# 0xC0000054/pdn-jpegxl

Hardware: AMD Instinct MI355X
Metric: megapixels/sec decode (4K lossy VarDCT) (higher is better)
Workload: dtype f32

## Files before the change

### pdn_jpegxl_amd/csrc/decoder.cc

```cpp
#include <hip/hip_runtime.h>
#include <algorithm>
#include <atomic>
#include <cmath>
#include <cstdarg>
#include <cstdio>
#include <cstdlib>
#include <cstring>
#include <memory>
#include <mutex>
#include <string>
#include <thread>
#include <vector>
#include "../../include/jxlfiletypeio.h"
#include "batch_layout.h"
#include "entropy_plan.h"
#include "host_parse.h"
#include "icc.h"
#include "kernels.h"

namespace jxlhip {

struct HipError : std::runtime_error {
  explicit HipError(const std::string& m) : std::runtime_error(m) {}
};
// ... 65 lines not shown
    std::vector<int> parse_status;
    std::vector<std::string> parse_msg;
    std::vector<size_t> status_off;
    DevImage* d_imgs = nullptr;
    bool pending = false;
    hipEvent_t lf_done = nullptr, hf_done = nullptr, done = nullptr, uploaded = nullptr;
    std::vector<Tap> taps;
    std::vector<std::string> stage_names;
    std::vector<int> stage_chain;
    std::vector<hipEvent_t> events;
    std::vector<float> stage_ms;
  };
  static constexpr int kSlots = 3;
  static constexpr int kPixelChunk = 32;
  Slot slots[kSlots];
  int cur = 0, last = 0;
  Slot* active = &slots[0];
  hipStream_t stream_lf = nullptr;
  hipStream_t stream_hf = nullptr;
  hipStream_t last_stream = nullptr;
  std::vector<std::string> total_names;
  std::vector<double> total_ms;
  int total_batches = 0;
  std::string sticky_error;
  int sticky_status = 0;
  uint8_t* li_dev = nullptr; uint8_t* li_host = nullptr; size_t li_cap = 0;
  void EnsureLoadImageBuffers(size_t bytes);
  int lane_stride_override = 0;
  int hf_stride_override = 0;
  bool debug_taps = false;
  int band_first_row = 0, band_rows = 0;
  bool no_stream_pairs = false;
  bool no_lf_pipeline = false;
  int alpha_narrow_limit = 32767;
  bool no_direct = false, mod_lanes64 = false;
  bool overlap = true;
  int downscale = 1;

  explicit JxlHipDecoder(int dev);
  ~JxlHipDecoder();
  void EnsureWs(size_t bytes);
  void EnsureBlob(size_t bytes);
  void Mark(const char* name, hipStream_t s, int chain);
  void WaitSlot(Slot& S);
  Slot& Last() { return slots[last]; }
  void Decode(int32_t n_, const uint8_t* const* host_data, const size_t* sizes, const uint8_t* const* dev_data,
              uint8_t* const* dev_out, hipStream_t stream, bool sync, DecoderStatus* statuses, ErrorInfo* err);
  DecoderStatus Finish(DecoderStatus* statuses, ErrorInfo* err);
  void CopyPlaneTap(int stage);
  void PrepassSingle(ParsedFrame& f, const uint8_t* dev_file);
  EntropyPlanOptions PlanOptions() const;
};

JxlHipDecoder::JxlHipDecoder(int dev) {
  if (dev < 0) HIP_OK(hipGetDevice(&dev));
  device = dev;
  HIP_OK(hipSetDevice(device));
  int entropy_cus = 0, pixel_cus = 0;
  if (const char* e = Knob("JXLHIP_ENTROPY_CUS")) entropy_cus = std::min(256, std::max(0, atoi(e)));
  if (const char* e = Knob("JXLHIP_PIXEL_CUS")) pixel_cus = std::min(256, std::max(0, atoi(e)));
  auto masked_stream = [](hipStream_t* s, int first, int count) {
    uint32_t mask[8] = {0, 0, 0, 0, 0, 0, 0, 0};
    for (int i = first; i < first + count; i++) mask[i >> 5] |= 1u << (i & 31);
    HIP_OK(hipExtStreamCreateWithCUMask(s, 8, mask));
  };
  if (pixel_cus) masked_stream(&own_stream, 256 - pixel_cus, pixel_cus);
// ... 398 lines not shown
  if (any_alpha && !(skip_stages & 4))
    LaunchAlphaAns(d_imgs, B.alpha_tasks, nalpha_t, plan.alpha_stride, plan.alpha.Bytes(), plan.direct_alpha, plan.lean_mod,
                   alpha_narrow, s_hf);
  if (!ds || any_alpha) Mark("alpha_ans", s_hf, 1);
  if (debug_taps && !ds) {
    taps.assign(n, Tap());
    LaunchExpandCoefficients(d_imgs, n, true, B.max_tiles, stream);
    HIP_OK(hipStreamSynchronize(stream));
    CopyPlaneTap(0);
  }
  const bool finish_on_hf = s_hf == stream || debug_taps || !Knob("JXLHIP_ALPHA_FINISH_ON_PIX");
  if (finish_on_hf) {
    if (any_alpha && !(skip_stages & 4)) LaunchAlphaFinish(d_imgs, n, max_groups, alpha_narrow > 0, s_hf);
    if (!ds || any_alpha) Mark("alpha_finish", s_hf, 1);
  }
  if (s_hf != stream) {
    HIP_OK(hipEventRecord(S.hf_done, s_hf));
    HIP_OK(hipStreamWaitEvent(stream, S.hf_done, 0));
  }
  Mark("main_start", stream, 2);
  if (!finish_on_hf) {
    if (any_alpha && !(skip_stages & 4)) LaunchAlphaFinish(d_imgs, n, max_groups, alpha_narrow > 0, stream);
    Mark("alpha_finish", stream, 2);
  }
  hipStream_t s_pix = pix_on_hf ? s_hf : stream;
  if (ds && B.any_vardct) {
    if (any_alpha) LaunchAlphaReduce(d_imgs, n, B.max_ds_cells, s_pix);
    LaunchLfOutput(d_imgs, n, B.max_ds_cells, s_pix);
    Mark("lf_output", s_pix, 2);
  }
  for (int c0 = 0; c0 < (ds ? 0 : n); c0 += pixel_chunk) {
    const int cnt = std::min(pixel_chunk, n - c0);
    if (!(skip_stages & 8))
    LaunchReconTiles(d_imgs + c0, cnt, B.max_tiles, d_basis_all, d_basis_small, d_llf_scale, d_basis_mfma, s_pix);
    Mark("reconstruct", s_pix, 2);
    LaunchExpandCoefficients(d_imgs + c0, cnt, false, B.max_tiles, s_pix);
    LaunchGenericReconstruct(d_imgs + c0, cnt, d_basis_all, d_basis_small, d_llf_scale, s_pix);
    Mark("reconstruct_generic", s_pix, 2);
    if (debug_taps) { HIP_OK(hipStreamSynchronize(s_pix)); CopyPlaneTap(1); }
    if (any_noise && !(early_noise && c0 == 0)) { LaunchNoise(d_imgs + c0, cnt, max_groups, B.max_w, B.max_h, s_pix); Mark("noise", s_pix, 2); }
    if (!(skip_stages & 16))
    LaunchFilterTiles(d_imgs + c0, cnt, B.max_w, B.max_h, B.stage_mask, B.any_unfiltered, B.any_fused, B.any_fused2, s_pix);
    Mark("filters+output", s_pix, 2);
  }
  if (s_pix != stream) {
    HIP_OK(hipEventRecord(S.hf_done, s_pix));
    HIP_OK(hipStreamWaitEvent(stream, S.hf_done, 0));
  }
  if (nmod_t) {
    if (s_lf != stream) { HIP_OK(hipEventRecord(S.lf_done, s_lf)); HIP_OK(hipStreamWaitEvent(stream, S.lf_done, 0)); }
    LaunchModularAns(d_imgs, n, B.mod_tasks, nmod_t, plan.mod.Bytes(), plan.max_mod_groups,
                     plan.max_mod_coded, plan.mod_lanes, plan.mod_rb, plan.mod_wp_lds, plan.direct_mod, stream);
    for (auto& op : B.mod_ops) {
      if (op.kind == 3) LaunchModularPalette(op.a, op.b, op.out, op.nout, op.type, op.rw, op.rh, op.status, stream);
      else LaunchModularOp(op.kind, op.a, op.b, op.c, op.aw, op.ah, op.rw, op.rh, op.type, stream);
    }
    LaunchModularOut(d_imgs, n, B.max_mod_pixels, stream);
    if (ds) LaunchBoxReduce(d_imgs, n, B.max_ds_cells, stream);
    Mark("modular", stream, 2);
  }
  if (!patches.tiles.empty()) {
    LaunchPatches(B.patch_frames, B.patch_tiles, (int)patches.tiles.size(), B.patch_list, B.patch_pos, B.patch_refs, stream);
    Mark("patches", stream, 2);
  }
  if (!comps.empty()) {
    LaunchCompose(B.comp_imgs, B.comp_frames, (int)comps.size(), B.max_segments, stream);
    Mark("compose", stream, 2);
// ... 203 lines not shown
    return DecoderStatus_DecodeError;
  }
}

DecoderStatus jxlhip_finish(JxlHipDecoder* dec, DecoderStatus* statuses, ErrorInfo* err) {
  if (!dec) return DecoderStatus_NullParameter;
  try {
    return dec->Finish(statuses, err);
  } catch (const std::exception& e) {
    SetErr(err, "%s", e.what());
    return DecoderStatus_DecodeError;
  }
}

int32_t jxlhip_set_option(JxlHipDecoder* dec, const char* name, int32_t value) {
  if (!dec || !name) return 0;
  if (!strcmp(name, "debug_taps")) { dec->debug_taps = value != 0; return 1; }
  if (!strcmp(name, "query_pixel_chunk")) return JxlHipDecoder::kPixelChunk;
  if (!strcmp(name, "lane_stride")) { if (value != 0 && !PowerOfTwoUpTo64(value)) return 0; dec->lane_stride_override = value; return 1; }
  if (!strcmp(name, "band_first_row")) { if (value < 0) return 0; dec->band_first_row = value; return 1; }
  if (!strcmp(name, "band_rows")) { if (value < 0) return 0; dec->band_rows = value; return 1; }
  if (!strcmp(name, "no_direct")) { dec->no_direct = value != 0; return 1; }
  if (!strcmp(name, "alpha_narrow_limit")) { if (value < 0 || value > 32767) return 0; dec->alpha_narrow_limit = value; return 1; }
  if (!strcmp(name, "query_alpha_narrow_groups") || !strcmp(name, "query_alpha_redo_groups")) {
    JxlHipDecoder::Slot& S = dec->Last();
    if (S.pending || !S.h_status) return -1;
    const int word = name[12] == 'n' ? kStatusAlphaNarrow : kStatusAlphaRedo;
    int64_t sum = 0;
    for (int i = 0; i < S.n; i++) sum += S.h_status[(size_t)i * 16 + word];
    return (int32_t)std::min<int64_t>(sum, INT32_MAX);
  }
  if (!strcmp(name, "no_stream_pairs")) { dec->no_stream_pairs = value != 0; return 1; }
  if (!strcmp(name, "no_lf_pipeline")) { dec->no_lf_pipeline = value != 0; return 1; }
  if (!strcmp(name, "mod_lanes64")) { dec->mod_lanes64 = value != 0; return 1; }
  if (!strcmp(name, "overlap")) { dec->overlap = value != 0; return 1; }
  if (!strcmp(name, "downscale")) { if (value != 1 && value != 8) return 0; dec->downscale = value; return 1; }
  return 0;
}

size_t jxlhip_read_plane(JxlHipDecoder* dec, int32_t index, const char* name, int32_t channel, void* dst, size_t capacity) {
  if (!dec || !name) return 0;
  JxlHipDecoder::Slot& S = dec->Last();
  if (index < 0 || index >= S.n || S.pending) return 0;
  if (S.parse_status[index] != DecoderStatus_Ok) return 0;
  const DevImage& d = S.imgs[index];
  std::string nm(name);
  const size_t cells = (size_t)d.w8 * d.h8, pix = (size_t)d.wp * d.hp;
  const void* src = nullptr;
  size_t bytes = 0;
  bool host = false;
  const int c = std::min(2, std::max(0, channel));
  if (nm == "lf") { src = d.lf_final[c]; bytes = cells * 4; }
  else if (nm == "lf_quant") { src = d.lfq[c]; bytes = cells * 4; }
  else if (nm == "cellinfo") { src = d.cellinfo; bytes = cells * 4; }
  else if (nm == "raw_quant") { src = d.rawq; bytes = cells * 2; }
  else if (nm == "sharpness") { src = d.sharp; bytes = cells; }
  else if (nm == "ytox") { src = d.ytox; bytes = (size_t)d.wt * d.ht; }
  else if (nm == "ytob") { src = d.ytob; bytes = (size_t)d.wt * d.ht; }
  else if (nm == "alpha") { src = d.alpha; bytes = (size_t)d.w * d.h; }
  else if (nm == "inv_sigma") { src = d.inv_sigma; bytes = cells * 4; }
  else if (dec->debug_taps && (size_t)index < S.taps.size()) {
    host = true;
    if (nm == "qcoef") { src = S.taps[index].qcoef[c].data(); bytes = S.taps[index].qcoef[c].size(); }
    else if (nm == "xyb_idct") { src = S.taps[index].xyb_idct[c].data(); bytes = S.taps[index].xyb_idct[c].size(); }
    else if (nm == "xyb_filtered") { src = S.taps[index].xyb_filtered[c].data(); bytes = S.taps[index].xyb_filtered[c].size(); }
    else if (nm == "noise_rnd") { src = S.taps[index].noise_rnd[c].data(); bytes = S.taps[index].noise_rnd[c].size(); }
// ... 230 lines not shown
```

### pdn_jpegxl_amd/csrc/kernels.h

```cpp
#pragma once
#include <hip/hip_runtime.h>
#include "dev_types.h"

namespace jxlhip {

void LaunchLfAns(const DevImage* imgs, const SectionTask* tasks, int ntasks, int slots, size_t lds_bytes, int scalar_rows, bool lean, hipStream_t s);
void LaunchLfFinish(const DevImage* imgs, const SectionTask* tasks, int ntasks, bool pipeline, hipStream_t s);
void LaunchHfBlockList(const DevImage* imgs, int nimg, int max_groups, hipStream_t s);
void LaunchHfDecode(const DevImage* imgs, const SectionTask* tasks, int nwg, int threads, int lane_stride, size_t lds_bytes, size_t lane_bytes,
                    hipStream_t s);
void LaunchAlphaAns(const DevImage* imgs, const SectionTask* tasks, int nwg, int lane_stride, size_t lds_bytes, int scalar_rows, bool lean, int narrow_limit,
                    hipStream_t s);
void LaunchAlphaFinish(const DevImage* imgs, int nimg, int max_groups, bool narrow, hipStream_t s);
void LaunchModularAns(const DevImage* imgs, int nimg, const SectionTask* tasks, int ntasks, size_t lds_bytes, int max_sections, int max_coded,
                      int lanes, int rb_width, int wp_lds, int scalar_rows, hipStream_t s);
void LaunchModularOp(int kind, int32_t* a, int32_t* b, int32_t* c, int aw, int ah, int rw, int rh, int type, hipStream_t s);
void LaunchModularPalette(const int32_t* palette, const int32_t* index, int32_t* const* out, int nout, int nb_colors, int w, int h, uint32_t* status,
                          hipStream_t s);
void LaunchModularOut(const DevImage* imgs, int nimg, size_t max_pixels, hipStream_t s);
void LaunchOrient(const uint8_t* src, uint8_t* dst, int w, int h, int px_bytes, int orientation, hipStream_t s);
void LaunchLfPixelStages(const DevImage* imgs, int nimg, size_t max_cells, hipStream_t s);
void LaunchExpandCoefficients(const DevImage* imgs, int nimg, bool all_tiles, int max_tiles, hipStream_t s);
void LaunchGenericReconstruct(const DevImage* imgs, int nimg, const float* basis_all, const float* basis_small,
                              const float* llf_scale, hipStream_t s);
void LaunchReconTiles(const DevImage* imgs, int nimg, int max_tiles, const float* basis_all, const float* basis_small,
                      const float* llf_scale, const float* basis_mfma, hipStream_t s);
void LaunchFilterTiles(const DevImage* imgs, int nimg, int max_w, int max_h, int stage_mask, bool any_unfiltered,
                       int any_fused, int any_fused2, hipStream_t s);

void LaunchLfOutput(const DevImage* imgs, int nimg, size_t max_cells, hipStream_t s);
void LaunchAlphaReduce(const DevImage* imgs, int nimg, size_t max_cells, hipStream_t s);
void LaunchBoxReduce(const DevImage* imgs, int nimg, size_t max_cells, hipStream_t s);

void LaunchNoise(const DevImage* imgs, int nimg, int max_groups, int max_w, int max_h, hipStream_t s);

void LaunchCompose(const ComposeImage* imgs, const ComposeFrame* frames, int nimg, int max_segments, hipStream_t s);
void LaunchPatches(const PatchFrame* frames, const PatchTile* tiles, int ntiles, const int32_t* list, const PatchPos* pos, const PatchRef* refs,
                   hipStream_t s);

void LaunchStatusToHost(const uint32_t* src, uint32_t* dst_pinned, int nwords, hipStream_t s);
#ifdef JXLHIP_EXPERIMENTS
void LaunchInterference(int kind, int wg_per_cu, int lds_kb, float ms, float* scratch, size_t scratch_bytes, hipStream_t s);
#endif

}
```

### pdn_jpegxl_amd/csrc/tile_kernels.hip

```cpp
#include <hip/hip_runtime.h>
#include <cstdlib>
#include "dev_types.h"
#include "dev_util.h"
#include "kernels.h"

namespace jxlhip {

#ifndef JXLHIP_PRIO_PIXEL
#define JXLHIP_PRIO_PIXEL 0
#endif
#if JXLHIP_PRIO_PIXEL
#define JXL_PIXEL_PRIO() __builtin_amdgcn_s_setprio(JXLHIP_PRIO_PIXEL)
#else
#define JXL_PIXEL_PRIO() ((void)0)
#endif

namespace {

constexpr int kTS = 64;
constexpr int kLP = 65;

__device__ const uint8_t t_quant_table[kNumStrategies] = {0, 1, 2, 3, 4, 5, 6, 6, 7, 7, 8, 8, 9, 9, 10, 10, 10, 10, 11, 12, 12, 13, 14, 14, 15, 16, 16};

__device__ __forceinline__ bool Special(uint32_t s) { return (s >= 1 && s <= 3) || (s >= 12 && s <= 17); }
typedef float __attribute__((ext_vector_type(4))) F4;
template <int N>
__device__ __forceinline__ F4 MfmaChain(const float* pa, int sa, const float* pb, int sb) {
  float a[N / 4], b[N / 4];
#pragma unroll
  for (int k = 0; k < N / 4; k++) { a[k] = pa[k * sa]; b[k] = pb[k * sb]; }
  F4 acc = {0.f, 0.f, 0.f, 0.f};
#pragma unroll
  for (int k = 0; k < N / 4; k++) acc = __builtin_amdgcn_mfma_f32_16x16x4f32(a[k], b[k], acc, 0, 0, 0);
  return acc;
}
template <bool kTableIsA>
__device__ __forceinline__ F4 MfmaChain32L(const float4* t_lo, const float4* t_hi, int pair, const float* po, int so) {
  const float4 v0 = t_lo[pair], v1 = t_hi[pair];
  const float t[8] = {v0.x, v0.y, v0.z, v0.w, v1.x, v1.y, v1.z, v1.w};
  float o[8];
#pragma unroll
  for (int k = 0; k < 8; k++) o[k] = po[k * so];
  F4 acc = {0.f, 0.f, 0.f, 0.f};
#pragma unroll
  for (int k = 0; k < 8; k++)
    acc = kTableIsA ? __builtin_amdgcn_mfma_f32_16x16x4f32(t[k], o[k], acc, 0, 0, 0) : __builtin_amdgcn_mfma_f32_16x16x4f32(o[k], t[k], acc, 0, 0, 0);
  return acc;
}
template <bool kTableIsA>
__device__ __forceinline__ F4 MfmaChain64L(const float4* t64, int pair, const float* po, int so) {
  float t[16], o[16];
#pragma unroll
  for (int j = 0; j < 4; j++) {
    const float4 v = t64[j * 256 + pair];
    t[4 * j] = v.x; t[4 * j + 1] = v.y; t[4 * j + 2] = v.z; t[4 * j + 3] = v.w;
  }
#pragma unroll
  for (int k = 0; k < 16; k++) o[k] = po[k * so];
  F4 acc = {0.f, 0.f, 0.f, 0.f};
#pragma unroll
  for (int k = 0; k < 16; k++)
    acc = kTableIsA ? __builtin_amdgcn_mfma_f32_16x16x4f32(t[k], o[k], acc, 0, 0, 0) : __builtin_amdgcn_mfma_f32_16x16x4f32(o[k], t[k], acc, 0, 0, 0);
  return acc;
}
__device__ __forceinline__ bool MfmaRows(uint32_t tl, uint32_t tr) {
  return (tl >> 31) && (tr >> 31) && ((tl >> 21) & 7) >= 1 && ((tl >> 21) & 7) == ((tr >> 21) & 7) && ((tl >> 13) & 31) == ((tr >> 13) & 31);
}
__device__ __forceinline__ bool MfmaCols(uint32_t tl, uint32_t bl) {
  return (tl >> 31) && (bl >> 31) && ((tl >> 18) & 7) >= 1 && ((tl >> 18) & 7) == ((bl >> 18) & 7) && ((tl >> 8) & 31) == ((bl >> 8) & 31);
}

__device__ __forceinline__ float SrgbOetfT(float v) {
  const float lin = 12.92f * v;
  const float cur = 1.055f * __builtin_amdgcn_exp2f(__builtin_amdgcn_logf(v) * (1.0f / 2.4f)) - 0.055f;
  return v <= 0.0031308f ? lin : cur;
}
__device__ __forceinline__ float SrgbOetf255T(float v) {
  const float lin = (12.92f * 255.0f) * v;
  const float cur = (1.055f * 255.0f) * __builtin_amdgcn_exp2f(__builtin_amdgcn_logf(v) * (1.0f / 2.4f)) - (0.055f * 255.0f);
  return v <= 0.0031308f ? lin : cur;
}
__device__ __forceinline__ float PowT(float a, float e) { return __builtin_amdgcn_exp2f(__builtin_amdgcn_logf(a) * e); }
__device__ __forceinline__ float EncodeTransferT(int kind, float v, float pq_scale, const float* lut = nullptr) {
  if (kind == 0) return v;
  if (kind == 5) {
    const float t = __builtin_sqrtf(fminf(fmaxf(v, 0.f), 1.f)) * 4095.0f;
    const int i = min((int)t, 4094);
    return lut[i] + (lut[i + 1] - lut[i]) * (t - (float)i);
  }
  const float a = fabsf(v);
  float r;
  if (kind == 1) r = a <= 0.0031308f ? 12.92f * a : 1.055f * PowT(a, 1.0f / 2.4f) - 0.055f;
  else if (kind == 2) r = a < 0.018f ? 4.5f * a : 1.099f * PowT(a, 0.45f) - 0.099f;
  else {
    const float xp = a > 0.f ? PowT(a * pq_scale, 0.1593017578125f) : 0.f;
// ... 104 lines not shown
    }
  }
  WritePixelA(im, x, y, X, Y, B, a);
}
__device__ __forceinline__ void WritePixel(const DevImage& im, int x, int y, float X, float Y, float B) {
  const uint32_t a = im.has_alpha ? LoadAlpha(im, (size_t)y * im.w + x) : 0u;
  if (im.has_noise) { WritePixelGeneral(im, x, y, X, Y, B, a); return; }
  WritePixelA(im, x, y, X, Y, B, a);
}

}

#define JXL_IDCT_STEP(Bp, v0, v1)                                                                  \
  {                                                                                                \
    const float4 b0 = *(const float4*)(Bp);                                                        \
    const float4 b1 = *(const float4*)((Bp) + 4);                                                  \
    a0[0] += v0 * b0.x; a0[1] += v0 * b0.y; a0[2] += v0 * b0.z; a0[3] += v0 * b0.w;                \
    a0[4] += v0 * b1.x; a0[5] += v0 * b1.y; a0[6] += v0 * b1.z; a0[7] += v0 * b1.w;                \
    a1[0] += v1 * b0.x; a1[1] += v1 * b0.y; a1[2] += v1 * b0.z; a1[3] += v1 * b0.w;                \
    a1[4] += v1 * b1.x; a1[5] += v1 * b1.y; a1[6] += v1 * b1.z; a1[7] += v1 * b1.w;                \
  }

__device__ __forceinline__ float DequantBias(int32_t v, float qb, float qb3) {
  if (v == 0) return 0.f;
  if (v == 1) return qb;
  if (v == -1) return -qb;
  const float f = (float)v;
  return f - qb3 * __builtin_amdgcn_rcpf(f);
}
typedef int __attribute__((ext_vector_type(4))) I4v;

constexpr int kTileF = kTS * kLP;

__global__ __launch_bounds__(768, 6) void recon_tile_kernel(const DevImage* __restrict__ imgs, const float* basis_all, const float* basis_small,
                                                             const float* llf_scale, const float* basis_mfma) {
  JXL_PIXEL_PRIO();
  extern __shared__ __align__(16) uint8_t smem_raw[];
  float* cfc3 = (float*)smem_raw;
  float* B816 = cfc3 + 3 * kTileF;
  float* cscale = B816 + 320;
  uint32_t* ci = (uint32_t*)(cscale + 64);
  uint32_t* cmeta = ci + 64;
  uint32_t* cnq = cmeta + 64;
  uint32_t* cpre = cnq + 64;
  uint32_t* cstart = cpre + 3 * 64;
  uint32_t* ctot = cstart + 3 * 64;
  const U32x2** csc = (const U32x2**)(ctot + 4);
  float4* t32_lo = (float4*)(csc + 64);
  float4* t32_hi = t32_lo + 128;
  float4* t64 = t32_hi + 128;
  const DevImage& im = imgs[blockIdx.y];
  const int tile = blockIdx.x;
  if (tile >= im.wt * im.ht) return;
  const int tid = threadIdx.x;
  const int tx = tile % im.wt, ty = tile / im.wt;
  if (ty < im.dec_gy0 * 4 || ty >= im.dec_gy1 * 4) return;
  const int wave = tid >> 6, lane = tid & 63, team = wave >> 2, tw = wave & 3;
  const int c = team == 0 ? 1 : (team == 1 ? 0 : 2);
  const int wp = im.wp, hp = im.hp;
  {
    float4* z = (float4*)cfc3;
    for (int i = tid; i < 3 * kTileF / 4; i += 768) z[i] = make_float4(0.f, 0.f, 0.f, 0.f);
  }
  int bad = 0, has64 = 0;
  if (tid < 64) {
    const int cx = tx * 8 + (tid & 7), cy = ty * 8 + (tid >> 3);
    const bool inside = cx < im.w8 && cy < im.h8;
    const size_t cell_g = (size_t)min(cy, im.h8 - 1) * im.w8 + min(cx, im.w8 - 1);
    const size_t ncells = (size_t)im.w8 * im.h8;
    const uint32_t info_g = im.cellinfo[cell_g];
    const uint32_t rq_g = im.rawq[cell_g];
    U32x2 blk[3];
    blk[0] = im.cblk[ncells + cell_g]; blk[1] = im.cblk[cell_g]; blk[2] = im.cblk[2 * ncells + cell_g];
    const uint32_t info = inside ? info_g : 0u;
    const uint32_t rqv = inside ? rq_g : 1u;
    const int ix = (info >> 8) & 31, iy = (info >> 13) & 31, lcx = (info >> 18) & 7, lcy = (info >> 21) & 7;
    if (inside) {
      if (!(info >> 31)) bad = 1;
      else {
        const int ox = (tid & 7) - ix, oy = (tid >> 3) - iy;
        bad = ox < 0 || oy < 0 || ox + (1 << lcx) > 8 || oy + (1 << lcy) > 8 || Special(info & 0xFF) ||
              (ox & ((1 << lcx) - 1)) != 0 || (oy & ((1 << lcy) - 1)) != 0;
      }
    }
    const bool valid = (info >> 31) && !bad;
    has64 = valid && (lcx == 3 || lcy == 3);
    {
      const uint64_t any = __ballot(has64);
      if (tid == 0) ctot[3] = any != 0;
    }
    const uint32_t q = t_quant_table[valid ? (info & 0xFF) : 0];
    const uint32_t rq_origin = (uint32_t)__shfl((int)rqv, valid ? tid - iy * 8 - ix : tid);
    const uint32_t lng = 3 + max(lcx, lcy);
    const bool transposed = lcy >= lcx;
    ci[tid] = info;
// ... 40 lines not shown
  }
  const float* const Bl = basis_all;
  float* const cfc = cfc3 + team * kTileF;
  if (tw == 0) {
    const int cxg = tx * 8 + (lane & 7), cyg = ty * 8 + (lane >> 3);
    const bool inside = cxg < im.w8 && cyg < im.h8;
    const float lf_g = im.lf_final[c][(size_t)min(cyg, im.h8 - 1) * im.w8 + min(cxg, im.w8 - 1)];
    const float lfv = inside ? lf_g : 0.f;
    const uint32_t info = ci[lane];
    const bool valid = info >> 31;
    const int ix = (info >> 8) & 31, iy = (info >> 13) & 31, lcx = (info >> 18) & 7, lcy = (info >> 21) & 7;
    const int cx = 1 << lcx, cy = 1 << lcy;
    const int ox = (lane & 7) - ix, oy = (lane >> 3) - iy;
    const float* Bx = basis_small + (cx * cx - 1) / 3 + ix * cx;
    const float* By = basis_small + (cy * cy - 1) / 3 + iy * cy;
    float bx[8], byv[8];
#pragma unroll
    for (int k = 0; k < 8; k++) { bx[k] = (valid && k < cx) ? Bx[k] : 0.f; byv[k] = (valid && k < cy) ? By[k] : 0.f; }
    const float sc = valid ? llf_scale[lcy * 32 + iy] * llf_scale[lcx * 32 + ix] / (float)(cx * cy) : 0.f;
    float row = 0.f;
#pragma unroll
    for (int k = 0; k < 8; k++) {
      const float v = __shfl(lfv, (lane - ix + k) & 63);
      if (valid && k < cx) row += v * bx[k];
    }
    float acc = 0.f;
#pragma unroll
    for (int k = 0; k < 8; k++) {
      const float v = __shfl(row, ((oy + k) * 8 + (lane & 7)) & 63);
      if (valid && k < cy) acc += v * byv[k];
    }
    if (valid) atomicAdd(&cfc[(oy * 8 + iy) * kLP + ox * 8 + ix], acc * sc);
  }
  {
    const size_t tile_cfl = (size_t)ty * im.wt + tx;
    const float cfl_x = im.base_x + (float)im.ytox[tile_cfl] * im.inv_color_factor;
    const float cfl_b = im.base_b + (float)im.ytob[tile_cfl] * im.inv_color_factor;
    const uint32_t* entries = im.centries + (size_t)((ty >> 2) * im.xg + (tx >> 2) - im.centries_g0) * kGroupEntriesCap;
    const uint32_t t0 = ctot[0], t01 = t0 + ctot[1], total = t01 + ctot[2];
    const float qb3 = im.qbias[3];
    for (uint32_t e = (uint32_t)tid; e < total; e += 768) {
      const uint32_t t = (e >= t0) + (e >= t01);
      const uint32_t el = e - (t == 0 ? 0u : (t == 1 ? t0 : t01));
      const uint32_t* pre = cpre + t * 64;
      uint32_t j = 0;
#pragma unroll
      for (int step = 32; step; step >>= 1) if (pre[j + step] <= el) j += step;
      const uint32_t ent = entries[cstart[t * 64 + j] + (el - pre[j])];
      const uint32_t k = ent & 0xFFFFu, nq = cnq[j];
      if (k >= nq) continue;
      const int chan = t == 0 ? 1 : (t == 1 ? 0 : 2);
      const U32x2 se = csc[j][(size_t)chan * nq + k];
      const uint32_t meta = cmeta[j];
      const uint32_t lng = meta & 15, p = se.x;
      const uint32_t r = p >> lng, cc = p & ((1u << lng) - 1);
      const uint32_t ky = (meta & 16) ? cc : r, kx = (meta & 16) ? r : cc;
      if (ky >= 64 || kx >= 64) continue;
      const int32_t v = (int32_t)ent >> 16;
      const float dm = t == 0 ? 1.0f : (t == 1 ? im.x_dm : im.b_dm);
      const float o = DequantBias(v, im.qbias[chan], qb3) * (cscale[j] * dm) * __uint_as_float(se.y);
      const uint32_t at = ((j >> 3) * 8 + ky) * kLP + (j & 7) * 8 + kx;
      atomicAdd(&cfc3[t * kTileF + at], o);
      if (t == 0) {
        if (cfl_x != 0.f) atomicAdd(&cfc3[kTileF + at], o * cfl_x);
        if (cfl_b != 0.f) atomicAdd(&cfc3[2 * kTileF + at], o * cfl_b);
      }
    }
  }
  __syncthreads();
  const int l16 = tid & 15, lq = lane >> 4;
  {
    F4 acc[4];
    bool m[4];
    const int x0 = tw * 16;
#pragma unroll
    for (int rb = 0; rb < 4; rb++) {
      const uint32_t inf = ci[rb * 16 + tw * 2];
      m[rb] = MfmaRows(inf, ci[rb * 16 + tw * 2 + 1]);
      if (m[rb]) {
        const int iy = (inf >> 13) & 31, lcy = (inf >> 21) & 7, R = 8 << lcy;
        const float* cp = cfc + ((rb * 2 - iy) * 8 + lq) * kLP + x0 + l16;
        if (R == 16) acc[rb] = MfmaChain<16>(B816 + 64 + lq * 16 + iy * 8 + l16, 64, cp, 4 * kLP);
        else if (R == 32) acc[rb] = MfmaChain32L<true>(t32_lo, t32_hi, (iy * 8 + l16) * 4 + lq, cp, 4 * kLP);
        else acc[rb] = MfmaChain64L<true>(t64, (iy * 8 + l16) * 4 + lq, cp, 4 * kLP);
      }
    }
    const int x = x0 + (lane & 7) * 2, cr = lane >> 3;
    const uint32_t info = ci[cr * 8 + (x >> 3)];
    const bool valu = (info >> 31) && !MfmaRows(ci[(cr >> 1) * 16 + (x >> 4) * 2], ci[(cr >> 1) * 16 + (x >> 4) * 2 + 1]);
    float a0[8] = {0, 0, 0, 0, 0, 0, 0, 0}, a1[8] = {0, 0, 0, 0, 0, 0, 0, 0};
    if (valu) {
      const int iy = (info >> 13) & 31, lcy = (info >> 21) & 7;
      const int R = 8 << lcy;
      const float* in = cfc + (cr - iy) * 8 * kLP + x;
      if (R == 8) {
#pragma unroll 2
        for (int k = 0; k < 8; k++) { const float v0 = in[k * kLP], v1 = in[k * kLP + 1]; JXL_IDCT_STEP(B816 + k * 8, v0, v1) }
      } else if (R == 16) {
        const float* B = B816 + 64 + iy * 8;
#pragma unroll 2
        for (int k = 0; k < 16; k++) { const float v0 = in[k * kLP], v1 = in[k * kLP + 1]; JXL_IDCT_STEP(B + k * 16, v0, v1) }
      } else {
        const float* B = Bl + (R * R - 64) / 3 + iy * 8;
        for (int k = 0; k < R; k++) { const float v0 = in[k * kLP], v1 = in[k * kLP + 1]; JXL_IDCT_STEP(B + k * R, v0, v1) }
      }
    }
    __builtin_amdgcn_fence(__ATOMIC_RELEASE, "wavefront");
    __builtin_amdgcn_wave_barrier();
#pragma unroll
    for (int rb = 0; rb < 4; rb++)
      if (m[rb]) {
        float* o = cfc + (rb * 16 + 4 * lq) * kLP + x0 + l16;
        o[0] = acc[rb].x; o[kLP] = acc[rb].y; o[2 * kLP] = acc[rb].z; o[3 * kLP] = acc[rb].w;
      }
    if (valu) {
#pragma unroll
      for (int j = 0; j < 8; j++) { cfc[(cr * 8 + j) * kLP + x] = a0[j]; cfc[(cr * 8 + j) * kLP + x + 1] = a1[j]; }
    }
  }
  __syncthreads();
  {
    F4 acc[4];
    bool m[4];
    const int y0 = tw * 16;
#pragma unroll
    for (int cs = 0; cs < 4; cs++) {
      const uint32_t inf = ci[tw * 16 + cs * 2];
      m[cs] = MfmaCols(inf, ci[tw * 16 + 8 + cs * 2]);
      if (m[cs]) {
        const int ix = (inf >> 8) & 31, lcx = (inf >> 18) & 7, C = 8 << lcx;
        const float* ap = cfc + (y0 + l16) * kLP + (cs * 2 - ix) * 8 + lq;
        if (C == 16) acc[cs] = MfmaChain<16>(ap, 4, B816 + 64 + lq * 16 + ix * 8 + l16, 64);
        else if (C == 32) acc[cs] = MfmaChain32L<false>(t32_lo, t32_hi, (ix * 8 + l16) * 4 + lq, ap, 4);
        else acc[cs] = MfmaChain64L<false>(t64, (ix * 8 + l16) * 4 + lq, ap, 4);
      }
    }
    const int y = y0 + (lane & 7) * 2, cc = lane >> 3;
    const uint32_t info = ci[(y >> 3) * 8 + cc];
    const bool valu = (info >> 31) && !MfmaCols(ci[(y >> 4) * 16 + (cc >> 1) * 2], ci[(y >> 4) * 16 + 8 + (cc >> 1) * 2]);
    float a0[8] = {0, 0, 0, 0, 0, 0, 0, 0}, a1[8] = {0, 0, 0, 0, 0, 0, 0, 0};
    if (valu) {
      const int ix = (info >> 8) & 31, lcx = (info >> 18) & 7;
      const int C = 8 << lcx;
      const float* in = cfc + y * kLP + (cc - ix) * 8;
      if (C == 8) {
#pragma unroll 2
        for (int k = 0; k < 8; k++) { const float v0 = in[k], v1 = in[k + kLP]; JXL_IDCT_STEP(B816 + k * 8, v0, v1) }
      } else if (C == 16) {
        const float* B = B816 + 64 + ix * 8;
#pragma unroll 2
        for (int k = 0; k < 16; k++) { const float v0 = in[k], v1 = in[k + kLP]; JXL_IDCT_STEP(B + k * 16, v0, v1) }
      } else {
        const float* B = Bl + (C * C - 64) / 3 + ix * 8;
        for (int k = 0; k < C; k++) { const float v0 = in[k], v1 = in[k + kLP]; JXL_IDCT_STEP(B + k * C, v0, v1) }
      }
    }
    __builtin_amdgcn_fence(__ATOMIC_RELEASE, "wavefront");
    __builtin_amdgcn_wave_barrier();
#pragma unroll
    for (int cs = 0; cs < 4; cs++)
      if (m[cs]) {
        float* o = cfc + (y0 + 4 * lq) * kLP + cs * 16 + l16;
        o[0] = acc[cs].x; o[kLP] = acc[cs].y; o[2 * kLP] = acc[cs].z; o[3 * kLP] = acc[cs].w;
      }
    if (valu) {
#pragma unroll
      for (int j = 0; j < 8; j++) { cfc[y * kLP + cc * 8 + j] = a0[j]; cfc[(y + 1) * kLP + cc * 8 + j] = a1[j]; }
// ... 679 lines not shown
  if (!im.ds || im.is_modular) return;
  const size_t n = (size_t)im.ds_w * im.ds_h;
  const float* __restrict__ pX = im.lf_final[0];
  const float* __restrict__ pY = im.lf_final[1];
  const float* __restrict__ pB = im.lf_final[2];
  const size_t gid = (size_t)blockIdx.x * blockDim.x + threadIdx.x, stride = (size_t)gridDim.x * blockDim.x;
  const bool quads = PlainOutput(im) && im.ds_orient == 1 && im.ncolor == 3 && ((uintptr_t)im.out & 15) == 0;
  if (!quads) {
    for (size_t i = gid; i < n; i += stride) LfOutputPixel(im, i, pX[i], pY[i], pB[i]);
    return;
  }
  const size_t nq = n >> 2;
  for (size_t q = gid; q < nq; q += stride) {
    const float4 X = ((const float4*)pX)[q], Y = ((const float4*)pY)[q], B = ((const float4*)pB)[q];
    const uint32_t a = im.has_alpha ? ((const uint32_t*)im.ds_alpha)[q] : 0u;
    const uint32_t p0 = PixelToRgba8(im, X.x, Y.x, B.x, a & 0xFF), p1 = PixelToRgba8(im, X.y, Y.y, B.y, (a >> 8) & 0xFF);
    const uint32_t p2 = PixelToRgba8(im, X.z, Y.z, B.z, (a >> 16) & 0xFF), p3 = PixelToRgba8(im, X.w, Y.w, B.w, a >> 24);
    if (im.nch_out == 4) ((uint4*)im.out)[q] = make_uint4(p0, p1, p2, p3);
    else ((uint3*)im.out)[q] = make_uint3((p0 & 0xFFFFFFu) | (p1 << 24), ((p1 >> 8) & 0xFFFFu) | (p2 << 16), ((p2 >> 16) & 0xFFu) | (p3 << 8));
  }
  if (blockIdx.x == 0 && threadIdx.x < (n & 3)) {
    const size_t i = 4 * nq + threadIdx.x;
    LfOutputPixel(im, i, pX[i], pY[i], pB[i]);
  }
}

void LaunchLfOutput(const DevImage* imgs, int nimg, size_t max_cells, hipStream_t s) {
  if (nimg <= 0) return;
  const size_t b = std::min<size_t>((max_cells + 255) / 256, 2048);
  hipLaunchKernelGGL(lf_output_kernel, dim3((unsigned)std::max<size_t>(1, b), nimg), dim3(256), 0, s, imgs);
}

void LaunchReconTiles(const DevImage* imgs, int nimg, int max_tiles, const float* basis_all, const float* basis_small,
                      const float* llf_scale, const float* basis_mfma, hipStream_t s) {
  const size_t lds = (size_t)(3 * kTileF + 320 + 64 * 4 + 64 * 6 + 4 + 128 + 1024 + 4096) * 4;
  static bool raised = false;
  if (!raised) { (void)hipFuncSetAttribute((const void*)recon_tile_kernel, hipFuncAttributeMaxDynamicSharedMemorySize, (int)lds); raised = true; }
  hipLaunchKernelGGL(recon_tile_kernel, dim3(max_tiles, nimg), dim3(768), lds, s, imgs, basis_all, basis_small, llf_scale, basis_mfma);
}

void LaunchFilterTiles(const DevImage* imgs, int nimg, int max_w, int max_h, int stage_mask, bool any_unfiltered,
                       int any_fused, int any_fused2, hipStream_t s) {
  const int tiles = ((max_w + 63) / 64) * ((max_h + 31) / 32);
  dim3 g(tiles, nimg);
  if (stage_mask & 1) hipLaunchKernelGGL(filter_tile_kernel<0>, g, dim3(256), 0, s, imgs);
  if (stage_mask & 2) hipLaunchKernelGGL(filter_tile_kernel<1>, g, dim3(256), 0, s, imgs);
  if (any_fused) {
    const int groups = ((max_w + kStripOut - 1) / kStripOut) * ((max_h + 2 + kSegRows - 1) / kSegRows);
    const int pair_groups = ((max_w + kPairOut - 1) / kPairOut) * ((max_h + 2 + kSegRows - 1) / kSegRows);
    if (any_fused & 1) hipLaunchKernelGGL(filter_stream_pairs_kernel, dim3((pair_groups + kGroupsPerWg - 1) / kGroupsPerWg, nimg), dim3(256), 0, s, imgs);
    if (any_fused & 2) hipLaunchKernelGGL(filter_stream_kernel, dim3((groups + kGroupsPerWg - 1) / kGroupsPerWg, nimg), dim3(256), 0, s, imgs);
    const int pair2_groups = ((max_w + kPair2Out - 1) / kPair2Out) * ((max_h + kSegRows - 1) / kSegRows);
    if (any_fused2 & 1) hipLaunchKernelGGL(filter_stream2_pairs_kernel, dim3((pair2_groups + kGroupsPerWg - 1) / kGroupsPerWg, nimg), dim3(256), 0, s, imgs);
    if (any_fused2 & 2) hipLaunchKernelGGL(filter_stream2_kernel, dim3((groups + kGroupsPerWg - 1) / kGroupsPerWg, nimg), dim3(256), 0, s, imgs);
  }
  if (stage_mask & 4) hipLaunchKernelGGL(filter_tile_kernel<2>, g, dim3(256), 0, s, imgs);
  if (stage_mask & 8) hipLaunchKernelGGL(filter_tile_kernel<3>, g, dim3(256), 0, s, imgs);
  if (any_unfiltered) {
    size_t work = (size_t)max_w * max_h;
    size_t b = std::min<size_t>((work + 255) / 256, 8192);
    hipLaunchKernelGGL(out_only_kernel, dim3((unsigned)b, nimg), dim3(256), 0, s, imgs);
  }
}

}
```

Baseline: 33500.

## Skip zero high-frequency MFMA steps in large-transform IDCT using coefficient extent masks

Tracks, per varblock and channel, which 4-row/4-column coefficient bands received nonzero coefficients, using an LDS bitmask filled with atomicOr during dequantization. The row and column MFMA passes for 16/32/64-point transforms then truncate their chains to the highest nonzero band, or skip a pass entirely when it has no coefficients. This is meant to cut MFMA and LDS-load work for sparse lossy blocks. In exchange it adds an atomic per coefficient, extra LDS, readfirstlane uniformity, and a runtime-variable chain length built with recursive templates. A recon_dense option disables the skipping.

```diff
diff --git a/pdn_jpegxl_amd/csrc/decoder.cc b/pdn_jpegxl_amd/csrc/decoder.cc
--- a/pdn_jpegxl_amd/csrc/decoder.cc
+++ b/pdn_jpegxl_amd/csrc/decoder.cc
@@ -121,6 +121,7 @@
   int band_first_row = 0, band_rows = 0;
   bool no_stream_pairs = false;
   bool no_lf_pipeline = false;
+  bool recon_dense = false;
   int alpha_narrow_limit = 32767;
   bool no_direct = false, mod_lanes64 = false;
   bool overlap = true;
@@ -585,7 +586,7 @@
   for (int c0 = 0; c0 < (ds ? 0 : n); c0 += pixel_chunk) {
     const int cnt = std::min(pixel_chunk, n - c0);
     if (!(skip_stages & 8))
-    LaunchReconTiles(d_imgs + c0, cnt, B.max_tiles, d_basis_all, d_basis_small, d_llf_scale, d_basis_mfma, s_pix);
+    LaunchReconTiles(d_imgs + c0, cnt, B.max_tiles, d_basis_all, d_basis_small, d_llf_scale, d_basis_mfma, recon_dense, s_pix);
     Mark("reconstruct", s_pix, 2);
     LaunchExpandCoefficients(d_imgs + c0, cnt, false, B.max_tiles, s_pix);
     LaunchGenericReconstruct(d_imgs + c0, cnt, d_basis_all, d_basis_small, d_llf_scale, s_pix);
@@ -855,6 +856,7 @@
   }
   if (!strcmp(name, "no_stream_pairs")) { dec->no_stream_pairs = value != 0; return 1; }
   if (!strcmp(name, "no_lf_pipeline")) { dec->no_lf_pipeline = value != 0; return 1; }
+  if (!strcmp(name, "recon_dense")) { dec->recon_dense = value != 0; return 1; }
   if (!strcmp(name, "mod_lanes64")) { dec->mod_lanes64 = value != 0; return 1; }
   if (!strcmp(name, "overlap")) { dec->overlap = value != 0; return 1; }
   if (!strcmp(name, "downscale")) { if (value != 1 && value != 8) return 0; dec->downscale = value; return 1; }
diff --git a/pdn_jpegxl_amd/csrc/kernels.h b/pdn_jpegxl_amd/csrc/kernels.h
--- a/pdn_jpegxl_amd/csrc/kernels.h
+++ b/pdn_jpegxl_amd/csrc/kernels.h
@@ -24,7 +24,7 @@
 void LaunchGenericReconstruct(const DevImage* imgs, int nimg, const float* basis_all, const float* basis_small,
                               const float* llf_scale, hipStream_t s);
 void LaunchReconTiles(const DevImage* imgs, int nimg, int max_tiles, const float* basis_all, const float* basis_small,
-                      const float* llf_scale, const float* basis_mfma, hipStream_t s);
+                      const float* llf_scale, const float* basis_mfma, bool dense, hipStream_t s);
 void LaunchFilterTiles(const DevImage* imgs, int nimg, int max_w, int max_h, int stage_mask, bool any_unfiltered,
                        int any_fused, int any_fused2, hipStream_t s);
 
diff --git a/pdn_jpegxl_amd/csrc/tile_kernels.hip b/pdn_jpegxl_amd/csrc/tile_kernels.hip
--- a/pdn_jpegxl_amd/csrc/tile_kernels.hip
+++ b/pdn_jpegxl_amd/csrc/tile_kernels.hip
@@ -24,43 +24,57 @@
 
 __device__ __forceinline__ bool Special(uint32_t s) { return (s >= 1 && s <= 3) || (s >= 12 && s <= 17); }
 typedef float __attribute__((ext_vector_type(4))) F4;
+template <int N> struct Regs { float v; Regs<N - 1> r; };
+template <> struct Regs<0> {};
+template <int K, int N>
+__device__ __forceinline__ float& Reg(Regs<N>& x) { if constexpr (K == 0) return x.v; else return Reg<K - 1>(x.r); }
+template <int K, int NK>
+__device__ __forceinline__ void ChainLoads(Regs<NK>& v, const float* p, int s, int n) {
+  if constexpr (K < NK) {
+    if (K == 0 || K < n) { Reg<K>(v) = p[K * s]; ChainLoads<K + 1, NK>(v, p, s, n); }
+  }
+}
+template <int K, int NK>
+__device__ __forceinline__ void ChainSteps(F4& acc, Regs<NK>& a, Regs<NK>& b, int n) {
+  if constexpr (K < NK) {
+    if (K == 0 || K < n) { acc = __builtin_amdgcn_mfma_f32_16x16x4f32(Reg<K>(a), Reg<K>(b), acc, 0, 0, 0); ChainSteps<K + 1, NK>(acc, a, b, n); }
+  }
+}
 template <int N>
-__device__ __forceinline__ F4 MfmaChain(const float* pa, int sa, const float* pb, int sb) {
-  float a[N / 4], b[N / 4];
-#pragma unroll
-  for (int k = 0; k < N / 4; k++) { a[k] = pa[k * sa]; b[k] = pb[k * sb]; }
+__device__ __forceinline__ F4 MfmaChain(const float* pa, int sa, const float* pb, int sb, int n) {
+  Regs<N / 4> a, b;
+  ChainLoads<0, N / 4>(a, pa, sa, n);
+  ChainLoads<0, N / 4>(b, pb, sb, n);
   F4 acc = {0.f, 0.f, 0.f, 0.f};
-#pragma unroll
-  for (int k = 0; k < N / 4; k++) acc = __builtin_amdgcn_mfma_f32_16x16x4f32(a[k], b[k], acc, 0, 0, 0);
+  ChainSteps<0, N / 4>(acc, a, b, n);
   return acc;
 }
+template <int J, int NK>
+__device__ __forceinline__ void ChainPieces(Regs<NK>& t, const float4* p, int stride, int n) {
+  if constexpr (4 * J < NK) {
+    if (J == 0 || 4 * J < n) {
+      const float4 v = p[J * stride];
+      Reg<4 * J>(t) = v.x; Reg<4 * J + 1>(t) = v.y; Reg<4 * J + 2>(t) = v.z; Reg<4 * J + 3>(t) = v.w;
+      ChainPieces<J + 1, NK>(t, p, stride, n);
+    }
+  }
+}
 template <bool kTableIsA>
-__device__ __forceinline__ F4 MfmaChain32L(const float4* t_lo, const float4* t_hi, int pair, const float* po, int so) {
-  const float4 v0 = t_lo[pair], v1 = t_hi[pair];
-  const float t[8] = {v0.x, v0.y, v0.z, v0.w, v1.x, v1.y, v1.z, v1.w};
-  float o[8];
-#pragma unroll
-  for (int k = 0; k < 8; k++) o[k] = po[k * so];
+__device__ __forceinline__ F4 MfmaChain32L(const float4* t_lo, const float4* t_hi, int pair, const float* po, int so, int n) {
+  Regs<8> t, o;
+  ChainPieces<0, 8>(t, t_lo + pair, (int)(t_hi - t_lo), n);
+  ChainLoads<0, 8>(o, po, so, n);
   F4 acc = {0.f, 0.f, 0.f, 0.f};
-#pragma unroll
-  for (int k = 0; k < 8; k++)
-    acc = kTableIsA ? __builtin_amdgcn_mfma_f32_16x16x4f32(t[k], o[k], acc, 0, 0, 0) : __builtin_amdgcn_mfma_f32_16x16x4f32(o[k], t[k], acc, 0, 0, 0);
+  if (kTableIsA) ChainSteps<0, 8>(acc, t, o, n); else ChainSteps<0, 8>(acc, o, t, n);
   return acc;
 }
 template <bool kTableIsA>
-__device__ __forceinline__ F4 MfmaChain64L(const float4* t64, int pair, const float* po, int so) {
-  float t[16], o[16];
-#pragma unroll
-  for (int j = 0; j < 4; j++) {
-    const float4 v = t64[j * 256 + pair];
-    t[4 * j] = v.x; t[4 * j + 1] = v.y; t[4 * j + 2] = v.z; t[4 * j + 3] = v.w;
-  }
-#pragma unroll
-  for (int k = 0; k < 16; k++) o[k] = po[k * so];
+__device__ __forceinline__ F4 MfmaChain64L(const float4* t64, int pair, const float* po, int so, int n) {
+  Regs<16> t, o;
+  ChainPieces<0, 16>(t, t64 + pair, 256, n);
+  ChainLoads<0, 16>(o, po, so, n);
   F4 acc = {0.f, 0.f, 0.f, 0.f};
-#pragma unroll
-  for (int k = 0; k < 16; k++)
-    acc = kTableIsA ? __builtin_amdgcn_mfma_f32_16x16x4f32(t[k], o[k], acc, 0, 0, 0) : __builtin_amdgcn_mfma_f32_16x16x4f32(o[k], t[k], acc, 0, 0, 0);
+  if (kTableIsA) ChainSteps<0, 16>(acc, t, o, n); else ChainSteps<0, 16>(acc, o, t, n);
   return acc;
 }
 __device__ __forceinline__ bool MfmaRows(uint32_t tl, uint32_t tr) {
@@ -231,8 +245,14 @@
 
 constexpr int kTileF = kTS * kLP;
 
+__device__ __forceinline__ uint32_t ExtentWord(const uint32_t* own, const uint32_t* luma, int origin, int lcx, int lcy, uint32_t dense) {
+  const uint32_t w = own[origin] | luma[origin] | (lcy == 3 ? 3u : 1u) | (lcx == 3 ? 0x30000u : 0x10000u) | dense;
+  return (uint32_t)__builtin_amdgcn_readfirstlane((int)w);
+}
+__device__ __forceinline__ uint32_t Uniform(uint32_t v) { return (uint32_t)__builtin_amdgcn_readfirstlane((int)v); }
+
 __global__ __launch_bounds__(768, 6) void recon_tile_kernel(const DevImage* __restrict__ imgs, const float* basis_all, const float* basis_small,
-                                                             const float* llf_scale, const float* basis_mfma) {
+                                                             const float* llf_scale, const float* basis_mfma, uint32_t dense) {
   JXL_PIXEL_PRIO();
   extern __shared__ __align__(16) uint8_t smem_raw[];
   float* cfc3 = (float*)smem_raw;
@@ -244,7 +264,8 @@
   uint32_t* cpre = cnq + 64;
   uint32_t* cstart = cpre + 3 * 64;
   uint32_t* ctot = cstart + 3 * 64;
-  const U32x2** csc = (const U32x2**)(ctot + 4);
+  uint32_t* cext = ctot + 4;
+  const U32x2** csc = (const U32x2**)(cext + 3 * 64);
   float4* t32_lo = (float4*)(csc + 64);
   float4* t32_hi = t32_lo + 128;
   float4* t64 = t32_hi + 128;
@@ -260,6 +281,7 @@
   {
     float4* z = (float4*)cfc3;
     for (int i = tid; i < 3 * kTileF / 4; i += 768) z[i] = make_float4(0.f, 0.f, 0.f, 0.f);
+    if (tid >= 768 - 3 * 64) cext[tid - (768 - 3 * 64)] = 0u;
   }
   int bad = 0, has64 = 0;
   if (tid < 64) {
@@ -366,10 +388,10 @@
     }
     if (valid) atomicAdd(&cfc[(oy * 8 + iy) * kLP + ox * 8 + ix], acc * sc);
   }
+  const size_t tile_cfl = (size_t)ty * im.wt + tx;
+  const float cfl_x = im.base_x + (float)im.ytox[tile_cfl] * im.inv_color_factor;
+  const float cfl_b = im.base_b + (float)im.ytob[tile_cfl] * im.inv_color_factor;
   {
-    const size_t tile_cfl = (size_t)ty * im.wt + tx;
-    const float cfl_x = im.base_x + (float)im.ytox[tile_cfl] * im.inv_color_factor;
-    const float cfl_b = im.base_b + (float)im.ytob[tile_cfl] * im.inv_color_factor;
     const uint32_t* entries = im.centries + (size_t)((ty >> 2) * im.xg + (tx >> 2) - im.centries_g0) * kGroupEntriesCap;
     const uint32_t t0 = ctot[0], t01 = t0 + ctot[1], total = t01 + ctot[2];
     const float qb3 = im.qbias[3];
@@ -394,6 +416,7 @@
       const float dm = t == 0 ? 1.0f : (t == 1 ? im.x_dm : im.b_dm);
       const float o = DequantBias(v, im.qbias[chan], qb3) * (cscale[j] * dm) * __uint_as_float(se.y);
       const uint32_t at = ((j >> 3) * 8 + ky) * kLP + (j & 7) * 8 + kx;
+      atomicOr(&cext[t * 64 + j], (1u << (ky >> 2)) | (1u << (16 + (kx >> 2))));
       atomicAdd(&cfc3[t * kTileF + at], o);
       if (t == 0) {
         if (cfl_x != 0.f) atomicAdd(&cfc3[kTileF + at], o * cfl_x);
@@ -403,20 +426,28 @@
   }
   __syncthreads();
   const int l16 = tid & 15, lq = lane >> 4;
+  const uint32_t* const ext_own = cext + team * 64;
+  const uint32_t* const ext_luma = (team == 1 ? cfl_x != 0.f : (team == 2 && cfl_b != 0.f)) ? cext : ext_own;
   {
     F4 acc[4];
     bool m[4];
     const int x0 = tw * 16;
 #pragma unroll
     for (int rb = 0; rb < 4; rb++) {
-      const uint32_t inf = ci[rb * 16 + tw * 2];
-      m[rb] = MfmaRows(inf, ci[rb * 16 + tw * 2 + 1]);
+      const uint32_t inf = Uniform(ci[rb * 16 + tw * 2]), inr = Uniform(ci[rb * 16 + tw * 2 + 1]);
+      m[rb] = MfmaRows(inf, inr);
       if (m[rb]) {
         const int iy = (inf >> 13) & 31, lcy = (inf >> 21) & 7, R = 8 << lcy;
+        const int ixl = (inf >> 8) & 31, ixr = (inr >> 8) & 31, orow = (rb * 2 - iy) * 8 + tw * 2;
+        const uint32_t wl = ExtentWord(ext_own, ext_luma, orow - ixl, (inf >> 18) & 7, lcy, dense);
+        const uint32_t wr = ExtentWord(ext_own, ext_luma, orow + 1 - ixr, (inr >> 18) & 7, lcy, dense);
+        const uint32_t rows = ((((wl >> (16 + 2 * ixl)) & 3) ? wl : 0u) | (((wr >> (16 + 2 * ixr)) & 3) ? wr : 0u)) & 0xFFFFu;
+        if (rows == 0) { m[rb] = false; continue; }
+        const int n = min(R / 4, 32 - __builtin_clz(rows));
         const float* cp = cfc + ((rb * 2 - iy) * 8 + lq) * kLP + x0 + l16;
-        if (R == 16) acc[rb] = MfmaChain<16>(B816 + 64 + lq * 16 + iy * 8 + l16, 64, cp, 4 * kLP);
-        else if (R == 32) acc[rb] = MfmaChain32L<true>(t32_lo, t32_hi, (iy * 8 + l16) * 4 + lq, cp, 4 * kLP);
-        else acc[rb] = MfmaChain64L<true>(t64, (iy * 8 + l16) * 4 + lq, cp, 4 * kLP);
+        if (R == 16) acc[rb] = MfmaChain<16>(B816 + 64 + lq * 16 + iy * 8 + l16, 64, cp, 4 * kLP, n);
+        else if (R == 32) acc[rb] = MfmaChain32L<true>(t32_lo, t32_hi, (iy * 8 + l16) * 4 + lq, cp, 4 * kLP, n);
+        else acc[rb] = MfmaChain64L<true>(t64, (iy * 8 + l16) * 4 + lq, cp, 4 * kLP, n);
       }
     }
     const int x = x0 + (lane & 7) * 2, cr = lane >> 3;
@@ -459,14 +490,18 @@
     const int y0 = tw * 16;
 #pragma unroll
     for (int cs = 0; cs < 4; cs++) {
-      const uint32_t inf = ci[tw * 16 + cs * 2];
-      m[cs] = MfmaCols(inf, ci[tw * 16 + 8 + cs * 2]);
+      const uint32_t inf = Uniform(ci[tw * 16 + cs * 2]), inb = Uniform(ci[tw * 16 + 8 + cs * 2]);
+      m[cs] = MfmaCols(inf, inb);
       if (m[cs]) {
         const int ix = (inf >> 8) & 31, lcx = (inf >> 18) & 7, C = 8 << lcx;
+        const int ocol = cs * 2 - ix, iyt = (inf >> 13) & 31, iyb = (inb >> 13) & 31;
+        const uint32_t wt = ExtentWord(ext_own, ext_luma, (tw * 2 - iyt) * 8 + ocol, lcx, (inf >> 21) & 7, dense);
+        const uint32_t wb = ExtentWord(ext_own, ext_luma, (tw * 2 + 1 - iyb) * 8 + ocol, lcx, (inb >> 21) & 7, dense);
+        const int n = min(C / 4, 32 - __builtin_clz((wt | wb) >> 16));
         const float* ap = cfc + (y0 + l16) * kLP + (cs * 2 - ix) * 8 + lq;
-        if (C == 16) acc[cs] = MfmaChain<16>(ap, 4, B816 + 64 + lq * 16 + ix * 8 + l16, 64);
-        else if (C == 32) acc[cs] = MfmaChain32L<false>(t32_lo, t32_hi, (ix * 8 + l16) * 4 + lq, ap, 4);
-        else acc[cs] = MfmaChain64L<false>(t64, (ix * 8 + l16) * 4 + lq, ap, 4);
+        if (C == 16) acc[cs] = MfmaChain<16>(ap, 4, B816 + 64 + lq * 16 + ix * 8 + l16, 64, n);
+        else if (C == 32) acc[cs] = MfmaChain32L<false>(t32_lo, t32_hi, (ix * 8 + l16) * 4 + lq, ap, 4, n);
+        else acc[cs] = MfmaChain64L<false>(t64, (ix * 8 + l16) * 4 + lq, ap, 4, n);
       }
     }
     const int y = y0 + (lane & 7) * 2, cc = lane >> 3;
@@ -1212,11 +1247,11 @@
 }
 
 void LaunchReconTiles(const DevImage* imgs, int nimg, int max_tiles, const float* basis_all, const float* basis_small,
-                      const float* llf_scale, const float* basis_mfma, hipStream_t s) {
-  const size_t lds = (size_t)(3 * kTileF + 320 + 64 * 4 + 64 * 6 + 4 + 128 + 1024 + 4096) * 4;
+                      const float* llf_scale, const float* basis_mfma, bool dense, hipStream_t s) {
+  const size_t lds = (size_t)(3 * kTileF + 320 + 64 * 4 + 64 * 6 + 64 * 3 + 4 + 128 + 1024 + 4096) * 4;
   static bool raised = false;
   if (!raised) { (void)hipFuncSetAttribute((const void*)recon_tile_kernel, hipFuncAttributeMaxDynamicSharedMemorySize, (int)lds); raised = true; }
-  hipLaunchKernelGGL(recon_tile_kernel, dim3(max_tiles, nimg), dim3(768), lds, s, imgs, basis_all, basis_small, llf_scale, basis_mfma);
+  hipLaunchKernelGGL(recon_tile_kernel, dim3(max_tiles, nimg), dim3(768), lds, s, imgs, basis_all, basis_small, llf_scale, basis_mfma, dense ? ~0u : 0u);
 }
 
 void LaunchFilterTiles(const DevImage* imgs, int nimg, int max_w, int max_h, int stage_mask, bool any_unfiltered,
```

Result: no change. 33760, median of 3 (+0.8%).
